# l90lpa/fv3-jedi-linearmodel

Hardware: AMD Instinct MI355X
Metric: column-updates/s per TL+AD dyn step (higher is better)
Workload: dtype f64; 1 GPU; C192L127 hydrostatic TL+AD, six cube faces dealt over 1 GPU(s) (6 per rank), table-driven exchange (221184 columns per GPU), k_split=2 n_split=6 dt=450s nq=4, hord mt/vt/tm/dp/tr=2/2/2/2/2 (sponge: 1/1/1/1 below level 9), kord=17, nord=1; columns_per_gpu=221184

## Files before the change

### fv3_jedi_linearmodel_amd/csrc/remap.h

```cpp
#pragma once
#include "column.h"

namespace fv3 {

struct ColWs {
  double* base; size_t stride; int kw;
  HD double& at(int slot, int k) const { return base[((size_t)slot * kw + k) * stride]; }
};
template <class T> struct WsIO;
template <> struct WsIO<double> {
  static constexpr int W = 1;
  HD static double get(const ColWs& w, int s, int k) { return w.at(s, k); }
  HD static void set(const ColWs& w, int s, int k, double x) { w.at(s, k) = x; }
};
template <> struct WsIO<Dual> {
  static constexpr int W = 2;
  HD static Dual get(const ColWs& w, int s, int k) { return Dual(w.at(2 * s, k), w.at(2 * s + 1, k)); }
  HD static void set(const ColWs& w, int s, int k, const Dual& x) { w.at(2 * s, k) = x.v; w.at(2 * s + 1, k) = x.d; }
};

constexpr double R3 = 1. / 3., R23 = 2. / 3.;

template <class T, class FP1, class FQ1, class FP2, class FOut>
HD void map_col(int km, const FP1& pe1, const FQ1& q1, const FP2& pe2, const FOut& out, const ColWs& ws, int SG, int SE) {
  typedef WsIO<T> W;
  T dpa = pe1(2) - pe1(1), dpb = pe1(3) - pe1(2);
  T grat = dpb / dpa;
  T bet = grat * (grat + 0.5);
  T qf = ((grat + grat) * (grat + 1.) * q1(1) + q1(2)) / bet;
  T gam = (1. + grat * (grat + 1.5)) / bet;
  W::set(ws, SE, 1, qf); W::set(ws, SG, 1, gam);
  T d4 = grat, a_prev = q1(1), dp_prev = dpa;
  for (int k = 2; k <= km; ++k) {
    T dpk = pe1(k + 1) - pe1(k);
    T ak_ = q1(k);
    d4 = dp_prev / dpk;
    bet = 2. + d4 + d4 - gam;
    qf = (3. * (a_prev + d4 * ak_) - qf) / bet;
    gam = d4 / bet;
    W::set(ws, SE, k, qf); W::set(ws, SG, k, gam);
    a_prev = ak_; dp_prev = dpk;
  }
  T a_bot = 1. + d4 * (d4 + 1.5);
  T qe = (2. * d4 * (d4 + 1.) * q1(km) + q1(km - 1) - a_bot * qf) / (d4 * (d4 + 0.5) - a_bot * gam);
  W::set(ws, SE, km + 1, qe);
  for (int k = km; k >= 1; --k) {
    qe = W::get(ws, SE, k) - W::get(ws, SG, k) * qe;
    W::set(ws, SE, k, qe);
  }
  int k0 = 1;
  T qsum = T(0.);
  for (int k = 1; k <= km; ++k) {
    const T p2t = pe2(k), p2b = pe2(k + 1);
    int l; bool found = false;
    for (l = k0; l <= km; ++l)
      if (val(p2t) >= val(pe1(l)) && val(p2t) <= val(pe1(l + 1))) { found = true; break; }
    if (found) {
      const T p1l = pe1(l), p1r = pe1(l + 1), dpl = p1r - p1l;
      const T a1 = q1(l), a2 = W::get(ws, SE, l), a3 = W::get(ws, SE, l + 1), a4 = 3. * (2. * a1 - (a2 + a3));
      const T pl = (p2t - p1l) / dpl;
      if (val(p2b) <= val(p1r)) {
        const T pr = (p2b - p1l) / dpl;
        out(k, a2 + 0.5 * (a4 + a3 - a2) * (pr + pl) - a4 * R3 * (pr * (pr + pl) + pl * pl));
        k0 = l;
        continue;
      }
      qsum = (p1r - p2t) * (a2 + 0.5 * (a4 + a3 - a2) * (1. + pl) - a4 * (R3 * (1. + pl * (1. + pl))));
      int m; bool bottom = false;
      for (m = l + 1; m <= km; ++m) {
        if (val(p2b) > val(pe1(m + 1))) qsum = qsum + (pe1(m + 1) - pe1(m)) * q1(m);
        else { bottom = true; break; }
      }
      if (bottom) {
        const T p1m = pe1(m), dpm = pe1(m + 1) - p1m;
        const T b1 = q1(m), b2 = W::get(ws, SE, m), b3 = W::get(ws, SE, m + 1), b4 = 3. * (2. * b1 - (b2 + b3));
        const T dp = p2b - p1m, esl = dp / dpm;
        qsum = qsum + dp * (b2 + 0.5 * esl * (b3 - b2 + b4 * (1. - R23 * esl)));
        k0 = m;
      }
    }
    out(k, qsum / (p2b - p2t));
  }
}

HD void cs_limiters(bool extm, double a1, double& a2, double& a3, double& a4, int iv) {
  if (iv == 0) {
    if (a1 <= 0.) { a2 = a1; a3 = a1; a4 = 0.; }
    else if (fabs(a3 - a2) < -a4) {
      if (a1 + 0.25 * (a3 - a2) * (a3 - a2) / a4 + a4 * (1. / 12.) < 0.) {
        if (a1 < a3 && a1 < a2) { a3 = a1; a2 = a1; a4 = 0.; }
        else if (a3 > a2) { a4 = 3. * (a2 - a1); a3 = a2 - a4; }
        else { a4 = 3. * (a3 - a1); a2 = a3 - a4; }
      }
    }
    return;
  }
  const bool flat = (iv == 1) ? ((a1 - a2) * (a1 - a3) >= 0.) : extm;
  if (flat) { a2 = a1; a3 = a1; a4 = 0.; return; }
  const double da1 = a3 - a2, da2 = da1 * da1, a6da = a4 * da1;
  if (a6da < -da2) { a4 = 3. * (a2 - a1); a3 = a2 - a4; }
  else if (a6da > da2) { a4 = 3. * (a3 - a1); a2 = a3 - a4; }
}
struct LimProfile { int kord, iv; bool scalar; double qmin; };
template <class FA, class FE>
HD void lim_layer(const LimProfile& P, int k, int km, const FA& a1, const FE& qe, double& a2, double& a3, double& a4) {
  const int ak = P.kord < 0 ? -P.kord : P.kord, iv = P.iv;
  auto qlim = [&](int j) -> double {
    double q = qe(j);
    if (j <= 1 || j >= km + 1) return q;
    const double lo = fmin(a1(j - 1), a1(j)), hi = fmax(a1(j - 1), a1(j));
    if (j == 2 || j == km) return fmax(fmin(q, hi), lo);
    const double g1 = a1(j - 1) - a1(j - 2), g2 = a1(j + 1) - a1(j);
    if (g1 * g2 > 0.) return fmax(fmin(q, hi), lo);
    if (g1 > 0.) return fmax(q, lo);
    q = fmin(q, hi);
    return iv == 0 ? fmax(0., q) : q;
  };
  auto gam = [&](int j) { return a1(j) - a1(j - 1); };
  auto extm = [&](int j) -> bool {
    return gam(j) * gam(j + 1) < 0.;
  };
  const double a = a1(k);
  a2 = qlim(k); a3 = qlim(k + 1);
  if (k == 1 || k == km) {
    const bool ex = (a2 - a) * (a3 - a) > 0.;
    if (k == 1) {
      if (iv == 0) a2 = fmax(0., a2);
      else if (iv == -1) { if (a2 * a <= 0.) a2 = 0.; }
    } else {
      if (iv == 0) a3 = fmax(0., a3);
      else if (iv == -1) { if (a3 * a <= 0.) a3 = 0.; }
    }
    a4 = 3. * (2. * a - (a2 + a3));
    cs_limiters(ex, a, a2, a3, a4, 1);
    return;
  }
  if (k == 2 || k == km - 1) { a4 = 3. * (2. * a - (a2 + a3)); cs_limiters(extm(k), a, a2, a3, a4, 2); return; }
  const bool ex = extm(k), small = P.scalar && a < P.qmin;
  auto huynh = [&]() {
    const double pmp_1 = a - 2. * gam(k + 1), lac_1 = pmp_1 + 1.5 * gam(k + 2);
    a2 = fmin(fmax(a2, fmin(a, fmin(pmp_1, lac_1))), fmax(a, fmax(pmp_1, lac_1)));
    const double pmp_2 = a + 2. * gam(k), lac_2 = pmp_2 - 1.5 * gam(k - 1);
    a3 = fmin(fmax(a3, fmin(a, fmin(pmp_2, lac_2))), fmax(a, fmax(pmp_2, lac_2)));
  };
  if (ak == 9) {
    if (ex && (extm(k - 1) || extm(k + 1) || small)) { a2 = a; a3 = a; a4 = 0.; }
    else {
      a4 = 3. * (2. * a - (a2 + a3));
      if (fabs(a4) > fabs(a2 - a3)) { huynh(); a4 = 3. * (2. * a - (a2 + a3)); }
    }
  } else if (ak == 10) {
    if (ex) {
      if (small || extm(k - 1) || extm(k + 1)) { a2 = a; a3 = a; a4 = 0.; }
      else a4 = 6. * a - 3. * (a2 + a3);
    } else {
      a4 = 6. * a - 3. * (a2 + a3);
      if (fabs(a4) > fabs(a2 - a3)) { huynh(); a4 = 6. * a - 3. * (a2 + a3); }
    }
  } else if (ak == 8) {
    huynh(); a4 = 3. * (2. * a - (a2 + a3));
  } else if (ak == 12) {
    if (ex) { a2 = a; a3 = a; a4 = 0.; }
    else {
      a4 = 6. * a - 3. * (a2 + a3);
      if (fabs(a4) > fabs(a2 - a3)) { huynh(); a4 = 6. * a - 3. * (a2 + a3); }
    }
  } else if (ak == 13) {
    if (ex) {
      if (extm(k - 1) && extm(k + 1)) { a2 = a; a3 = a; a4 = 0.; }
      else { huynh(); a4 = 3. * (2. * a - (a2 + a3)); }
    } else a4 = 3. * (2. * a - (a2 + a3));
  } else if (ak == 14) {
    a4 = 3. * (2. * a - (a2 + a3));
  } else {
    if (ex && (extm(k - 1) || extm(k + 1) || small)) { a2 = a; a3 = a; a4 = 0.; }
    else a4 = 3. * (2. * a - (a2 + a3));
  }
  if (iv == 0) cs_limiters(ex, a, a2, a3, a4, 0);
}
template <class FP1, class FQ1, class FP2, class FE, class FOut>
HD void map_loop_lim(const LimProfile& P, int km, const FP1& pe1, const FQ1& q1, const FP2& pe2, const FE& qe, const FOut& out) {
  int k0 = 1;
  double qsum = 0.;
  for (int k = 1; k <= km; ++k) {
    const double p2t = pe2(k), p2b = pe2(k + 1);
    int l; bool found = false;
    for (l = k0; l <= km; ++l)
      if (p2t >= pe1(l) && p2t <= pe1(l + 1)) { found = true; break; }
    if (found) {
      const double p1l = pe1(l), p1r = pe1(l + 1), dpl = p1r - p1l;
      double a2, a3, a4; lim_layer(P, l, km, q1, qe, a2, a3, a4);
      const double pl = (p2t - p1l) / dpl;
      if (p2b <= p1r) {
        const double pr = (p2b - p1l) / dpl;
        out(k, a2 + 0.5 * (a4 + a3 - a2) * (pr + pl) - a4 * R3 * (pr * (pr + pl) + pl * pl));
        k0 = l;
        continue;
      }
      qsum = (p1r - p2t) * (a2 + 0.5 * (a4 + a3 - a2) * (1. + pl) - a4 * (R3 * (1. + pl * (1. + pl))));
      int m; bool bottom = false;
      for (m = l + 1; m <= km; ++m) {
        if (p2b > pe1(m + 1)) qsum = qsum + (pe1(m + 1) - pe1(m)) * q1(m);
        else { bottom = true; break; }
      }
      if (bottom) {
        const double p1m = pe1(m), dpm = pe1(m + 1) - p1m;
        double b2, b3, b4; lim_layer(P, m, km, q1, qe, b2, b3, b4);
        const double dp = p2b - p1m, esl = dp / dpm;
        qsum = qsum + dp * (b2 + 0.5 * esl * (b3 - b2 + b4 * (1. - R23 * esl)));
        k0 = m;
      }
    }
    out(k, qsum / (p2b - p2t));
  }
}

template <class FP1, class FQ1, class FP2, class FOut>
HD void map_col_lim(const LimProfile& P, int km, const FP1& pe1, const FQ1& q1, const FP2& pe2, const FOut& out, const ColWs& ws, int SG, int SE) {
  {
    double dpa = pe1(2) - pe1(1), dpb = pe1(3) - pe1(2);
    double grat = dpb / dpa, bet = grat * (grat + 0.5);
    double qf = ((grat + grat) * (grat + 1.) * q1(1) + q1(2)) / bet, gam = (1. + grat * (grat + 1.5)) / bet;
    ws.at(SE, 1) = qf; ws.at(SG, 1) = gam;
    double d4 = grat, a_prev = q1(1), dp_prev = dpa;
    for (int k = 2; k <= km; ++k) {
      const double dpk = pe1(k + 1) - pe1(k), ak_ = q1(k);
      d4 = dp_prev / dpk;
      bet = 2. + d4 + d4 - gam;
      qf = (3. * (a_prev + d4 * ak_) - qf) / bet;
      gam = d4 / bet;
      ws.at(SE, k) = qf; ws.at(SG, k) = gam;
      a_prev = ak_; dp_prev = dpk;
    }
    const double a_bot = 1. + d4 * (d4 + 1.5);
    double qe = (2. * d4 * (d4 + 1.) * q1(km) + q1(km - 1) - a_bot * qf) / (d4 * (d4 + 0.5) - a_bot * gam);
// ... 464 lines not shown
  typedef RemapAdSlots R_;
  auto pe1 = [&](int k) { return a.pe.t[fidx(g, a.pe, tile, i, j, k)]; };
  auto pn1 = [&](int k) { return a.peln.t[fidx(g, a.peln, tile, i, j, k)]; };
  auto pk1 = [&](int k) { return a.pk.t[fidx(g, a.pk, tile, i, j, k)]; };
  const double ps = pe1(km + 1);
  auto pe2 = [&](int k) -> double { return k == 1 ? a.ptop : (k == km + 1 ? ps : a.ak[k - 1] + a.bk[k - 1] * ps); };
  auto pn2 = [&](int k) -> double { return (k == 1 || k == km + 1) ? pn1(k) : log(pe2(k)); };
  auto pk2 = [&](int k) -> double { return (k == 1 || k == km + 1) ? pk1(k) : exp(a.akap * pn2(k)); };
  auto ptin = [&](int k) { return a.pt.t[fidx(g, a.pt, tile, i, j, k)]; };
  auto tv = [&](int k) -> double { return ptin(k) * (pk1(k + 1) - pk1(k)) / (a.akap * (pn1(k + 1) - pn1(k))); };
  for (int k = 0; k <= km + 1; ++k)
    for (int s_ : {R_::SPE1, R_::SPN1, R_::SPK1, R_::SPE2, R_::SPN2, R_::SPK2}) ws.at(s_, k) = 0.;
  {
    auto outT = [&](int k, double x) { ws.at(R_::ST2, k) = x; };
    bool done = false;
    if constexpr (LIM) if (kord_limited(a.kord_tm)) { map_col_lim(LimProfile{a.kord_tm, 1, true, 184.}, km, pn1, tv, pn2, outT, ws, 0, 1); done = true; }
    if (!done) map_col<double>(km, pn1, tv, pn2, outT, ws, 0, 1);
    if (a.nq > 0 && a.last_step) {
      auto q1 = [&](int k) { return a.q[0].t[fidx(g, a.q[0], tile, i, j, k)]; };
      auto outQ = [&](int k, double x) { ws.at(R_::SQ2, k) = x; };
      bool doneq = false;
      if constexpr (LIM) if (kord_limited(a.kord_tr)) { map_col_lim(LimProfile{a.kord_tr, 0, true, 0.}, km, pe1, q1, pe2, outQ, ws, 0, 1); doneq = true; }
      if (!doneq) map_col<double>(km, pe1, q1, pe2, outQ, ws, 0, 1);
    }
  }
  for (int k = 1; k <= km; ++k) {
    const size_t n0 = fidx(g, a.pt, tile, i, j, k);
    const double pk_hi = pk2(k), pk_lo = pk2(k + 1), pn_hi = pn2(k), pn_lo = pn2(k + 1);
    const double den = a.akap * (pn_lo - pn_hi), pkz = (pk_lo - pk_hi) / den;
    const double pt_ad = a.pt.p[n0], t2 = ws.at(R_::ST2, k);
    double pkz_ad = a.pkz.p[n0], t2_ad;
    if (a.last_step) {
      const double qv = a.nq > 0 ? ws.at(R_::SQ2, k) : 0., f = 1. + a.zvir * qv;
      t2_ad = pt_ad / f;
      if (a.nq > 0) a.q[0].p[fidx(g, a.q[0], tile, i, j, k)] += -(t2 / f) * a.zvir * pt_ad / f;
    } else {
      t2_ad = pt_ad / pkz;
      pkz_ad += -(t2 / pkz) * pt_ad / pkz;
    }
    ws.at(R_::SV, k) = t2_ad;
    const double za = pkz_ad / den;
    ws.at(R_::SPK2, k + 1) += za; ws.at(R_::SPK2, k) -= za;
    const double zb = -pkz * a.akap * za;
    ws.at(R_::SPN2, k + 1) += zb; ws.at(R_::SPN2, k) -= zb;
    const double dpa = a.delp.p[n0];
    ws.at(R_::SPE2, k + 1) += dpa; ws.at(R_::SPE2, k) -= dpa;
    a.delp.p[n0] = 0.; a.pkz.p[n0] = 0.;
  }
  for (int k = 2; k <= km; ++k) {
    ws.at(R_::SPK2, k) += a.pk.p[fidx(g, a.pk, tile, i, j, k)];
    ws.at(R_::SPN2, k) += a.peln.p[fidx(g, a.peln, tile, i, j, k)];
  }
}
HD void remap_ad_k2(const RemapArgs& a, int field, int i, int j, int tile, size_t col) {
  const Geom& g = a.g; const int km = g.npz;
  const ColWs ws{a.ws + col, a.ws_stride, km + 2};
  const FieldAdSlots S = remap_field_slots(field);
  auto pe1 = [&](int k) { return a.pe.t[fidx(g, a.pe, tile, i, j, k)]; };
  const double ps = pe1(km + 1);
  auto pe2 = [&](int k) -> double { return k == 1 ? a.ptop : (k == km + 1 ? ps : a.ak[k - 1] + a.bk[k - 1] * ps); };
  auto p1out = [&](int k, double x) { ws.at(S.SP1, k) = x; };
  auto p2out = [&](int k, double x) { ws.at(S.SP2, k) = x; };
  if (field == 0) {
    auto pn1 = [&](int k) { return a.peln.t[fidx(g, a.peln, tile, i, j, k)]; };
    auto pk1 = [&](int k) { return a.pk.t[fidx(g, a.pk, tile, i, j, k)]; };
    auto pn2 = [&](int k) -> double { return (k == 1 || k == km + 1) ? pn1(k) : log(pe2(k)); };
    auto tv = [&](int k) -> double { return a.pt.t[fidx(g, a.pt, tile, i, j, k)] * (pk1(k + 1) - pk1(k)) / (a.akap * (pn1(k + 1) - pn1(k))); };
    auto q2ad = [&](int k) { return ws.at(RemapAdSlots::SV, k); };
    map_col_ad_s(km, pn1, tv, pn2, q2ad, ws, S.w, [&](int k, double x) { ws.at(S.SQ1, k) = x; }, p1out, p2out);
  } else {
    const Fld& qf = a.q[field - 1];
    auto q1 = [&](int k) { return qf.t[fidx(g, qf, tile, i, j, k)]; };
    auto q2ad = [&](int k) { return qf.p[fidx(g, qf, tile, i, j, k)]; };
    map_col_ad_s(km, pe1, q1, pe2, q2ad, ws, S.w, [&](int k, double x) { qf.p[fidx(g, qf, tile, i, j, k)] = x; }, p1out, p2out);
  }
}
HD void remap_ad_k3(const RemapArgs& a, int i, int j, int tile, size_t col) {
  const Geom& g = a.g; const int km = g.npz;
  const ColWs ws{a.ws + col, a.ws_stride, km + 2};
  typedef RemapAdSlots R_;
  auto pe1 = [&](int k) { return a.pe.t[fidx(g, a.pe, tile, i, j, k)]; };
  auto pn1 = [&](int k) { return a.peln.t[fidx(g, a.peln, tile, i, j, k)]; };
  auto pk1 = [&](int k) { return a.pk.t[fidx(g, a.pk, tile, i, j, k)]; };
  const double ps = pe1(km + 1);
  auto pe2 = [&](int k) -> double { return k == 1 ? a.ptop : (k == km + 1 ? ps : a.ak[k - 1] + a.bk[k - 1] * ps); };
  auto pn2 = [&](int k) -> double { return (k == 1 || k == km + 1) ? pn1(k) : log(pe2(k)); };
  auto pk2 = [&](int k) -> double { return (k == 1 || k == km + 1) ? pk1(k) : exp(a.akap * pn2(k)); };
  {
    const FieldAdSlots S = remap_field_slots(0);
    for (int k = 1; k <= km + 1; ++k) { ws.at(R_::SPN1, k) += ws.at(S.SP1, k); ws.at(R_::SPN2, k) += ws.at(S.SP2, k); }
    for (int k = 1; k <= km; ++k) {
      const double tv_ad = ws.at(S.SQ1, k), dpk = pk1(k + 1) - pk1(k), den = a.akap * (pn1(k + 1) - pn1(k)), pt0 = a.pt.t[fidx(g, a.pt, tile, i, j, k)];
      a.pt.p[fidx(g, a.pt, tile, i, j, k)] = tv_ad * dpk / den;
      const double za = pt0 * tv_ad / den;
      ws.at(R_::SPK1, k + 1) += za; ws.at(R_::SPK1, k) -= za;
      const double zb = -(pt0 * dpk / den) * a.akap * tv_ad / den;
      ws.at(R_::SPN1, k + 1) += zb; ws.at(R_::SPN1, k) -= zb;
    }
  }
  for (int n = 0; n < a.nq; ++n) {
    const FieldAdSlots S = remap_field_slots(1 + n);
    for (int k = 1; k <= km + 1; ++k) { ws.at(R_::SPE1, k) += ws.at(S.SP1, k); ws.at(R_::SPE2, k) += ws.at(S.SP2, k); }
  }
  for (int k = 2; k <= km; ++k) {
    const double pn_ad = ws.at(R_::SPN2, k) + a.akap * pk2(k) * ws.at(R_::SPK2, k);
    ws.at(R_::SPE2, k) += pn_ad / pe2(k);
  }
  for (int k : {1, km + 1}) {
    ws.at(R_::SPN1, k) += ws.at(R_::SPN2, k) + a.peln.p[fidx(g, a.peln, tile, i, j, k)];
    ws.at(R_::SPK1, k) += ws.at(R_::SPK2, k) + a.pk.p[fidx(g, a.pk, tile, i, j, k)];
  }
  double ps_ad = ws.at(R_::SPE2, km + 1);
  for (int k = 2; k <= km; ++k) ps_ad += a.bk[k - 1] * ws.at(R_::SPE2, k);
  ws.at(R_::SPE1, km + 1) += ps_ad;
  for (int k = 1; k <= km + 1; ++k) {
    a.pk.p[fidx(g, a.pk, tile, i, j, k)] = ws.at(R_::SPK1, k);
    a.peln.p[fidx(g, a.peln, tile, i, j, k)] = ws.at(R_::SPN1, k);
    a.pe.p[fidx(g, a.pe, tile, i, j, k)] += ws.at(R_::SPE1, k);
  }
}

template <int MODE, bool LIM = false>
struct RemapFieldFn {
  RemapArgs a; int nf;
  HD void operator()(int i, int j, int z) const {
    const int tile = z / nf, field = z % nf;
    const size_t col = (size_t)tile * a.g.plane + a.g.idx(i, j);
    if (MODE == MODE_NL) remap_field_col<double, LIM>(a, field, i, j, tile, col);
    else if (MODE == MODE_TL) remap_field_col<Dual, LIM>(a, field, i, j, tile, col);
    else remap_ad_k2(a, field, i, j, tile, col);
  }
};
template <int MODE, bool LIM = false>
struct RemapPressFn {
  RemapArgs a;
  HD void operator()(int i, int j, int z) const {
    const size_t col = (size_t)z * a.g.plane + a.g.idx(i, j);
    if (MODE == MODE_NL) remap_press_col<double>(a, i, j, z);
    else if (MODE == MODE_TL) remap_press_col<Dual>(a, i, j, z);
    else if (MODE == MODE_AD) remap_ad_k1<LIM>(a, i, j, z, col);
    else remap_ad_k3(a, i, j, z, col);
  }
};
template <int MODE, bool LIM = false>
struct RemapWindFn {
  RemapArgs a; int dir;
  HD void operator()(int i, int j, int z) const {
    const size_t col = (size_t)z * a.g.plane + a.g.idx(i, j);
    if (MODE == MODE_NL) remap_wind_col<double, LIM>(a, dir, i, j, z, col);
    else if (MODE == MODE_TL) remap_wind_col<Dual, LIM>(a, dir, i, j, z, col);
    else remap_wind_col_ad(a, dir, i, j, z, col);
  }
};
inline void run_remap_winds(Exec& ex, int mode, const RemapArgs& a, double bytes = 0.) {
  const Geom& g = a.g;
  const Rect U{g.is(), g.ie(), g.js(), g.je() + 1}, V{g.is(), g.ie() + 1, g.js(), g.je()};
  if (kord_limited(a.kord_mt) && mode != MODE_AD) {
    if (mode == MODE_NL) { for_points(ex, U, g.ntile, RemapWindFn<MODE_NL, true>{a, 0}, "remap_wind_lim.nl", bytes); for_points(ex, V, g.ntile, RemapWindFn<MODE_NL, true>{a, 1}, "remap_wind_lim.nl", bytes); }
    else { for_points(ex, U, g.ntile, RemapWindFn<MODE_TL, true>{a, 0}, "remap_wind_lim.tl", bytes); for_points(ex, V, g.ntile, RemapWindFn<MODE_TL, true>{a, 1}, "remap_wind_lim.tl", bytes); }
  }
  else if (mode == MODE_NL) { for_points(ex, U, g.ntile, RemapWindFn<MODE_NL>{a, 0}, "remap_wind.nl", bytes); for_points(ex, V, g.ntile, RemapWindFn<MODE_NL>{a, 1}, "remap_wind.nl", bytes); }
  else if (mode == MODE_TL) { for_points(ex, U, g.ntile, RemapWindFn<MODE_TL>{a, 0}, "remap_wind.tl", bytes); for_points(ex, V, g.ntile, RemapWindFn<MODE_TL>{a, 1}, "remap_wind.tl", bytes); }
  else { for_points(ex, V, g.ntile, RemapWindFn<MODE_AD>{a, 1}, "remap_wind.ad", bytes); for_points(ex, U, g.ntile, RemapWindFn<MODE_AD>{a, 0}, "remap_wind.ad", bytes); }
}
struct RemapGatherFn {
  RemapArgs a;
  HD void operator()(int i, int j, int z) const { remap_pe_gather_ad(a, i, j, z); }
};
struct RemapPeFn {
  RemapArgs a; int mode;
  HD void operator()(int i, int j, int z) const {
    for (int k = 2; k <= a.g.npz; ++k) {
      const size_t n = fidx(a.g, a.pe, z, i, j, k);
      a.pe.t[n] = a.pe2.t[n];
      if (mode == MODE_TL) a.pe.p[n] = a.pe2.p[n];
    }
  }
};

inline int remap_ws_slots(int nq) { return RemapAdSlots::FBASE + RemapAdSlots::FN * (1 + nq); }
inline void run_remap(Exec& ex, int mode, const RemapArgs& a) {
  const Geom& g = a.g;
  const Rect A{g.is(), g.ie(), g.js(), g.je()}, H{g.is() - 1, g.ie() + 1, g.js() - 1, g.je() + 1};
  if (mode != MODE_AD) {
    const double cells = double(g.tx) * g.ty * g.ntile * g.npz, w = mode == MODE_TL ? 2. : 1.;
    const int nf = 1 + a.nq;
    const bool lim = kord_limited(a.kord_tm) || kord_limited(a.kord_tr);
    if (lim && mode == MODE_TL) {
      for_points(ex, A, g.ntile * nf, RemapFieldFn<MODE_TL, true>{a, nf}, "remap_fields_lim.tl", 8. * w * (5. + 2. * a.nq) * cells);
      for_points(ex, A, g.ntile, RemapPressFn<MODE_TL>{a}, "remap_press.tl", 8. * w * (5. + 7.) * cells);
    } else if (lim) {
      for_points(ex, A, g.ntile * nf, RemapFieldFn<MODE_NL, true>{a, nf}, "remap_fields_lim.nl", 8. * w * (5. + 2. * a.nq) * cells);
      for_points(ex, A, g.ntile, RemapPressFn<MODE_NL>{a}, "remap_press.nl", 8. * w * (5. + 7.) * cells);
    } else if (mode == MODE_TL) {
      for_points(ex, A, g.ntile * nf, RemapFieldFn<MODE_TL>{a, nf}, "remap_fields.tl", 8. * w * (5. + 2. * a.nq) * cells);
      for_points(ex, A, g.ntile, RemapPressFn<MODE_TL>{a}, "remap_press.tl", 8. * w * (5. + 7.) * cells);
    } else {
      for_points(ex, A, g.ntile * nf, RemapFieldFn<MODE_NL>{a, nf}, "remap_fields.nl", 8. * w * (5. + 2. * a.nq) * cells);
      for_points(ex, A, g.ntile, RemapPressFn<MODE_NL>{a}, "remap_press.nl", 8. * w * (5. + 7.) * cells);
    }
    run_remap_winds(ex, mode, a, 8. * w * 4. * cells);
    for_points(ex, A, g.ntile, RemapPeFn{a, mode}, "remap_pe");
  } else {
    const double cells = double(g.tx) * g.ty * g.ntile * g.npz;
    run_remap_winds(ex, MODE_AD, a, 8. * 7. * cells);
    for_points(ex, H, g.ntile, RemapGatherFn{a}, "remap_gather.ad", 8. * 4. * cells);
    const int nf = 1 + a.nq;
    if (kord_limited(a.kord_tm) || kord_limited(a.kord_tr)) for_points(ex, A, g.ntile, RemapPressFn<MODE_AD, true>{a}, "remap_scalars1_lim.ad", 8. * 12. * cells);
    else for_points(ex, A, g.ntile, RemapPressFn<MODE_AD>{a}, "remap_scalars1.ad", 8. * 12. * cells);
    for_points(ex, A, g.ntile * nf, RemapFieldFn<MODE_AD>{a, nf}, "remap_fields.ad", 8. * (4. + 3. * a.nq) * cells);
    for_points(ex, A, g.ntile, RemapPressFn<3>{a}, "remap_scalars3.ad", 8. * 8. * cells);
  }
}

}
```

Measured before the change: 184,400 column-updates/s.

## Split vertical remap into edge-solve and LDS-staged parallel per-level mapping kernels

Splits the per-column PPM remap for the NL/TL paths into two kernels: one computes edge values (batching up to four tracers per thread and sharing the tridiagonal coefficients), and one stages pressure, field and edge arrays for a strip of columns in LDS. In the second kernel, threads map each target level independently via binary search, so the serial per-column search loop goes away. Columns whose source or target pressures are not monotonic fall back to the serial mapping loop. This adds extra launches, workspace traffic and barrier synchronisation, in exchange for more parallelism and coalesced loads in the mapping step.

```diff
diff --git a/fv3_jedi_linearmodel_amd/csrc/remap.h b/fv3_jedi_linearmodel_amd/csrc/remap.h
--- a/fv3_jedi_linearmodel_amd/csrc/remap.h
+++ b/fv3_jedi_linearmodel_amd/csrc/remap.h
@@ -21,8 +21,8 @@
 
 constexpr double R3 = 1. / 3., R23 = 2. / 3.;
 
-template <class T, class FP1, class FQ1, class FP2, class FOut>
-HD void map_col(int km, const FP1& pe1, const FQ1& q1, const FP2& pe2, const FOut& out, const ColWs& ws, int SG, int SE) {
+template <class T, class FP1, class FQ1>
+HD void map_edges(int km, const FP1& pe1, const FQ1& q1, const ColWs& ws, int SG, int SE) {
   typedef WsIO<T> W;
   T dpa = pe1(2) - pe1(1), dpb = pe1(3) - pe1(2);
   T grat = dpb / dpa;
@@ -48,6 +48,81 @@
     qe = W::get(ws, SE, k) - W::get(ws, SG, k) * qe;
     W::set(ws, SE, k, qe);
   }
+}
+template <class T, int N, class FP1, class FQ1>
+HD void map_edges_n(int km, int nact, const FP1& pe1, const FQ1& q1, const ColWs& ws, int SG, int SE0) {
+  typedef WsIO<T> W;
+  T dpa = pe1(2) - pe1(1), dpb = pe1(3) - pe1(2);
+  T grat = dpb / dpa;
+  T bet = grat * (grat + 0.5);
+  T gam = (1. + grat * (grat + 1.5)) / bet;
+  T qf[N], a_prev[N];
+#pragma unroll
+  for (int n = 0; n < N; ++n) if (n < nact) {
+    a_prev[n] = q1(n, 1);
+    qf[n] = ((grat + grat) * (grat + 1.) * a_prev[n] + q1(n, 2)) / bet;
+    W::set(ws, SE0 + n, 1, qf[n]);
+  }
+  W::set(ws, SG, 1, gam);
+  T d4 = grat, dp_prev = dpa;
+  for (int k = 2; k <= km; ++k) {
+    T dpk = pe1(k + 1) - pe1(k);
+    d4 = dp_prev / dpk;
+    bet = 2. + d4 + d4 - gam;
+#pragma unroll
+    for (int n = 0; n < N; ++n) if (n < nact) {
+      T ak_ = q1(n, k);
+      qf[n] = (3. * (a_prev[n] + d4 * ak_) - qf[n]) / bet;
+      W::set(ws, SE0 + n, k, qf[n]);
+      a_prev[n] = ak_;
+    }
+    gam = d4 / bet;
+    W::set(ws, SG, k, gam);
+    dp_prev = dpk;
+  }
+  T a_bot = 1. + d4 * (d4 + 1.5);
+  T qe[N];
+#pragma unroll
+  for (int n = 0; n < N; ++n) if (n < nact) {
+    qe[n] = (2. * d4 * (d4 + 1.) * q1(n, km) + q1(n, km - 1) - a_bot * qf[n]) / (d4 * (d4 + 0.5) - a_bot * gam);
+    W::set(ws, SE0 + n, km + 1, qe[n]);
+  }
+  for (int k = km; k >= 1; --k) {
+    const T g = W::get(ws, SG, k);
+#pragma unroll
+    for (int n = 0; n < N; ++n) if (n < nact) {
+      qe[n] = W::get(ws, SE0 + n, k) - g * qe[n];
+      W::set(ws, SE0 + n, k, qe[n]);
+    }
+  }
+}
+template <class T, class FP1, class FQ1, class FSE>
+HD T map_target(int km, int l, const T& p2t, const T& p2b, const FP1& pe1, const FQ1& q1, const FSE& se, T& qsum, int& k0) {
+  const T p1l = pe1(l), p1r = pe1(l + 1), dpl = p1r - p1l;
+  const T a1 = q1(l), a2 = se(l), a3 = se(l + 1), a4 = 3. * (2. * a1 - (a2 + a3));
+  const T pl = (p2t - p1l) / dpl;
+  if (val(p2b) <= val(p1r)) {
+    const T pr = (p2b - p1l) / dpl;
+    k0 = l;
+    return a2 + 0.5 * (a4 + a3 - a2) * (pr + pl) - a4 * R3 * (pr * (pr + pl) + pl * pl);
+  }
+  qsum = (p1r - p2t) * (a2 + 0.5 * (a4 + a3 - a2) * (1. + pl) - a4 * (R3 * (1. + pl * (1. + pl))));
+  int m; bool bottom = false;
+  for (m = l + 1; m <= km; ++m) {
+    if (val(p2b) > val(pe1(m + 1))) qsum = qsum + (pe1(m + 1) - pe1(m)) * q1(m);
+    else { bottom = true; break; }
+  }
+  if (bottom) {
+    const T p1m = pe1(m), dpm = pe1(m + 1) - p1m;
+    const T b1 = q1(m), b2 = se(m), b3 = se(m + 1), b4 = 3. * (2. * b1 - (b2 + b3));
+    const T dp = p2b - p1m, esl = dp / dpm;
+    qsum = qsum + dp * (b2 + 0.5 * esl * (b3 - b2 + b4 * (1. - R23 * esl)));
+    k0 = m;
+  }
+  return qsum / (p2b - p2t);
+}
+template <class T, class FP1, class FQ1, class FP2, class FSE, class FOut>
+HD void map_loop(int km, const FP1& pe1, const FQ1& q1, const FP2& pe2, const FSE& se, const FOut& out) {
   int k0 = 1;
   T qsum = T(0.);
   for (int k = 1; k <= km; ++k) {
@@ -55,32 +130,14 @@
     int l; bool found = false;
     for (l = k0; l <= km; ++l)
       if (val(p2t) >= val(pe1(l)) && val(p2t) <= val(pe1(l + 1))) { found = true; break; }
-    if (found) {
-      const T p1l = pe1(l), p1r = pe1(l + 1), dpl = p1r - p1l;
-      const T a1 = q1(l), a2 = W::get(ws, SE, l), a3 = W::get(ws, SE, l + 1), a4 = 3. * (2. * a1 - (a2 + a3));
-      const T pl = (p2t - p1l) / dpl;
-      if (val(p2b) <= val(p1r)) {
-        const T pr = (p2b - p1l) / dpl;
-        out(k, a2 + 0.5 * (a4 + a3 - a2) * (pr + pl) - a4 * R3 * (pr * (pr + pl) + pl * pl));
-        k0 = l;
-        continue;
-      }
-      qsum = (p1r - p2t) * (a2 + 0.5 * (a4 + a3 - a2) * (1. + pl) - a4 * (R3 * (1. + pl * (1. + pl))));
-      int m; bool bottom = false;
-      for (m = l + 1; m <= km; ++m) {
-        if (val(p2b) > val(pe1(m + 1))) qsum = qsum + (pe1(m + 1) - pe1(m)) * q1(m);
-        else { bottom = true; break; }
-      }
-      if (bottom) {
-        const T p1m = pe1(m), dpm = pe1(m + 1) - p1m;
-        const T b1 = q1(m), b2 = W::get(ws, SE, m), b3 = W::get(ws, SE, m + 1), b4 = 3. * (2. * b1 - (b2 + b3));
-        const T dp = p2b - p1m, esl = dp / dpm;
-        qsum = qsum + dp * (b2 + 0.5 * esl * (b3 - b2 + b4 * (1. - R23 * esl)));
-        k0 = m;
-      }
-    }
-    out(k, qsum / (p2b - p2t));
-  }
+    if (found) out(k, map_target<T>(km, l, p2t, p2b, pe1, q1, se, qsum, k0));
+    else out(k, qsum / (p2b - p2t));
+  }
+}
+template <class T, class FP1, class FQ1, class FP2, class FOut>
+HD void map_col(int km, const FP1& pe1, const FQ1& q1, const FP2& pe2, const FOut& out, const ColWs& ws, int SG, int SE) {
+  map_edges<T>(km, pe1, q1, ws, SG, SE);
+  map_loop<T>(km, pe1, q1, pe2, [&](int k) { return WsIO<T>::get(ws, SE, k); }, out);
 }
 
 HD void cs_limiters(bool extm, double a1, double& a2, double& a3, double& a4, int iv) {
@@ -851,8 +908,13 @@
     else remap_wind_col_ad(a, dir, i, j, z, col);
   }
 };
+}
+#include "remap_split.h"
+namespace fv3 {
+
 inline void run_remap_winds(Exec& ex, int mode, const RemapArgs& a, double bytes = 0.) {
   const Geom& g = a.g;
+  if (mode != MODE_AD && !kord_limited(a.kord_mt) && run_remap_winds_split(ex, mode, a, bytes)) return;
   const Rect U{g.is(), g.ie(), g.js(), g.je() + 1}, V{g.is(), g.ie() + 1, g.js(), g.je()};
   if (kord_limited(a.kord_mt) && mode != MODE_AD) {
     if (mode == MODE_NL) { for_points(ex, U, g.ntile, RemapWindFn<MODE_NL, true>{a, 0}, "remap_wind_lim.nl", bytes); for_points(ex, V, g.ntile, RemapWindFn<MODE_NL, true>{a, 1}, "remap_wind_lim.nl", bytes); }
@@ -885,7 +947,10 @@
     const double cells = double(g.tx) * g.ty * g.ntile * g.npz, w = mode == MODE_TL ? 2. : 1.;
     const int nf = 1 + a.nq;
     const bool lim = kord_limited(a.kord_tm) || kord_limited(a.kord_tr);
-    if (lim && mode == MODE_TL) {
+    if (!lim && run_remap_fields_split(ex, mode, a, cells)) {
+      if (mode == MODE_TL) for_points(ex, A, g.ntile, RemapPressFn<MODE_TL>{a}, "remap_press.tl", 8. * w * (5. + 7.) * cells);
+      else for_points(ex, A, g.ntile, RemapPressFn<MODE_NL>{a}, "remap_press.nl", 8. * w * (5. + 7.) * cells);
+    } else if (lim && mode == MODE_TL) {
       for_points(ex, A, g.ntile * nf, RemapFieldFn<MODE_TL, true>{a, nf}, "remap_fields_lim.tl", 8. * w * (5. + 2. * a.nq) * cells);
       for_points(ex, A, g.ntile, RemapPressFn<MODE_TL>{a}, "remap_press.tl", 8. * w * (5. + 7.) * cells);
     } else if (lim) {
diff --git a/fv3_jedi_linearmodel_amd/csrc/remap_split.h b/fv3_jedi_linearmodel_amd/csrc/remap_split.h
--- /dev/null
+++ b/fv3_jedi_linearmodel_amd/csrc/remap_split.h
@@ -0,0 +1,259 @@
+#pragma once
+
+namespace fv3 {
+
+constexpr int RS_NT = 4;
+constexpr int RS_NTH = 512;
+constexpr int RS_CMAX = 64;
+inline bool remap_split_enabled() { const char* e = std::getenv("FV3LM_REMAP_SPLIT"); return !(e && e[0] == '0'); }
+inline size_t remap_split_lds(int npz, int C, bool tl) { return (size_t)3 * (npz + 2) * C * (tl ? 16 : 8); }
+inline int remap_split_cols(int npz, bool tl) {
+  int C = RS_CMAX;
+  while (C >= 8 && remap_split_lds(npz, C, tl) > 160 * 1024) C /= 2;
+  while (C >= 16 && remap_split_lds(npz, C, tl) > 53 * 1024) C /= 2;
+  return C >= 8 ? C : 0;
+}
+
+template <class T_>
+struct RsTv {
+  typedef T_ T; typedef FIO<T> IO;
+  const RemapArgs& a; int i, j, tile;
+  HD RsTv(const RemapArgs& a_, int, int i_, int j_, int tile_) : a(a_), i(i_), j(j_), tile(tile_) {}
+  HD static int nfld(const RemapArgs&) { return 1; }
+  HD static int slot_e(const RemapArgs&, int, int) { return 1; }
+  HD T pn1(int k) const { return IO::ld(a.peln, fidx(a.g, a.peln, tile, i, j, k)); }
+  HD T pk1(int k) const { return IO::ld(a.pk, fidx(a.g, a.pk, tile, i, j, k)); }
+  HD T pe1(int k) const { return pn1(k); }
+  HD T q1(int, int k) const { return IO::ld(a.pt, fidx(a.g, a.pt, tile, i, j, k)) * (pk1(k + 1) - pk1(k)) / (a.akap * (pn1(k + 1) - pn1(k))); }
+  HD T surf() const { return IO::ld(a.pe, fidx(a.g, a.pe, tile, i, j, a.g.npz + 1)); }
+  HD T pe2p(int k, const T& ps) const { const int km = a.g.npz; return k == 1 ? T(a.ptop) : (k == km + 1 ? ps : a.ak[k - 1] + a.bk[k - 1] * ps); }
+  HD T pe2(int k, const T& ps) const { return (k == 1 || k == a.g.npz + 1) ? pn1(k) : dlog(pe2p(k, ps)); }
+  HD void st(int, int k, const T& x) const { IO::st(a.pt, fidx(a.g, a.pt, tile, i, j, k), x); }
+};
+template <class T_>
+struct RsTr {
+  typedef T_ T; typedef FIO<T> IO;
+  const RemapArgs& a; int i, j, tile;
+  HD RsTr(const RemapArgs& a_, int, int i_, int j_, int tile_) : a(a_), i(i_), j(j_), tile(tile_) {}
+  HD static int nfld(const RemapArgs& a_) { return a_.nq; }
+  HD static int slot_e(const RemapArgs&, int, int n) { return 2 + n; }
+  HD T pe1(int k) const { return IO::ld(a.pe, fidx(a.g, a.pe, tile, i, j, k)); }
+  HD Fld qn(int n) const {
+    Fld f = a.q[0];
+#pragma unroll
+    for (int m = 1; m < 8; ++m) if (m == n) f = a.q[m];
+    return f;
+  }
+  HD T q1(int n, int k) const { const Fld f = qn(n); return IO::ld(f, fidx(a.g, f, tile, i, j, k)); }
+  HD T surf() const { return pe1(a.g.npz + 1); }
+  HD T pe2(int k, const T& ps) const { const int km = a.g.npz; return k == 1 ? T(a.ptop) : (k == km + 1 ? ps : a.ak[k - 1] + a.bk[k - 1] * ps); }
+  HD void st(int n, int k, const T& x) const { const Fld f = qn(n); IO::st(f, fidx(a.g, f, tile, i, j, k), x); }
+};
+template <class T_>
+struct RsWind {
+  typedef T_ T; typedef FIO<T> IO;
+  const RemapArgs& a; int dir, i, j, tile, im, jm;
+  HD RsWind(const RemapArgs& a_, int dir_, int i_, int j_, int tile_) : a(a_), dir(dir_), i(i_), j(j_), tile(tile_), im(dir_ == 0 ? i_ : i_ - 1), jm(dir_ == 0 ? j_ - 1 : j_) {}
+  HD static int nfld(const RemapArgs&) { return 1; }
+  HD static int slot_e(const RemapArgs&, int dir_, int) { return 2 * dir_ + 1; }
+  HD const Fld& wf() const { return dir == 0 ? a.u : a.v; }
+  HD T pe1(int k) const {
+    if (k == 1) return IO::ld(a.pe, fidx(a.g, a.pe, tile, i, j, 1));
+    return 0.5 * (IO::ld(a.pe, fidx(a.g, a.pe, tile, im, jm, k)) + IO::ld(a.pe, fidx(a.g, a.pe, tile, i, j, k)));
+  }
+  HD T q1(int, int k) const { return IO::ld(wf(), fidx(a.g, wf(), tile, i, j, k)); }
+  HD T surf() const { const int km = a.g.npz; return IO::ld(a.pe, fidx(a.g, a.pe, tile, im, jm, km + 1)) + IO::ld(a.pe, fidx(a.g, a.pe, tile, i, j, km + 1)); }
+  HD T pe2(int k, const T& pss) const { return (dir == 1 && k == 1) ? T(a.ak[0]) : a.ak[k - 1] + (0.5 * a.bk[k - 1]) * pss; }
+  HD void st(int, int k, const T& x) const { IO::st(wf(), fidx(a.g, wf(), tile, i, j, k), x); }
+};
+HD Rect remap_wind_rect(const Geom& g, int dir) { return dir == 0 ? Rect{g.is(), g.ie(), g.js(), g.je() + 1} : Rect{g.is(), g.ie() + 1, g.js(), g.je()}; }
+
+template <class T>
+struct RemapEdgesFieldFn {
+  RemapArgs a; int ng;
+  HD void operator()(int i, int j, int z) const {
+    const int tile = z / ng, grp = z % ng, km = a.g.npz;
+    const ColWs ws{a.ws + (size_t)tile * a.g.plane + a.g.idx(i, j), a.ws_stride, km + 2};
+    if (grp == 0) {
+      const RsTv<T> p(a, 0, i, j, tile);
+      map_edges<T>(km, [&](int k) { return p.pe1(k); }, [&](int k) { return p.q1(0, k); }, ws, 0, 1);
+    } else {
+      const RsTr<T> p(a, 0, i, j, tile);
+      const int n0 = RS_NT * (grp - 1), nact = a.nq - n0 < RS_NT ? a.nq - n0 : RS_NT;
+      map_edges_n<T, RS_NT>(km, nact, [&](int k) { return p.pe1(k); }, [&](int n, int k) { return p.q1(n0 + n, k); }, ws, 2 + a.nq + (grp - 1), 2 + n0);
+    }
+  }
+};
+template <class T>
+struct RemapEdgesWindFn {
+  RemapArgs a;
+  HD void operator()(int i, int j, int z) const {
+    const int tile = z / 2, dir = z % 2, km = a.g.npz;
+    if (!remap_wind_rect(a.g, dir).has(i, j)) return;
+    const ColWs ws{a.ws + (size_t)tile * a.g.plane + a.g.idx(i, j), a.ws_stride, km + 2};
+    const RsWind<T> p(a, dir, i, j, tile);
+    map_edges<T>(km, [&](int k) { return p.pe1(k); }, [&](int k) { return p.q1(0, k); }, ws, 2 * dir, 2 * dir + 1);
+  }
+};
+
+#ifdef FV3LM_HOST_EMUL
+DEV void rs_sync() {}
+#else
+DEV void rs_sync() { __syncthreads(); }
+#endif
+template <int U, class T, class FL, class FS>
+DEV void rs_stage(int n, int tid, int nth, const FL& ld, const FS& st) {
+  for (int e0 = tid; e0 < n; e0 += U * nth) {
+    T v[U];
+#pragma unroll
+    for (int u = 0; u < U; ++u) { const int e = e0 + u * nth; if (e < n) v[u] = ld(e); }
+#pragma unroll
+    for (int u = 0; u < U; ++u) { const int e = e0 + u * nth; if (e < n) st(e, v[u]); }
+  }
+}
+template <class PL>
+DEV void remap_map_block(const RemapArgs& a, int sel, const Rect& R, int tile, int j, int i0, int C, unsigned char* mem, int tid, int nth) {
+  typedef typename PL::T T; typedef WsIO<T> W;
+  const int km = a.g.npz, nc = R.i1 - i0 + 1 < C ? R.i1 - i0 + 1 : C, nf = PL::nfld(a);
+  int lc = 0; while ((1 << lc) < C) ++lc;
+  constexpr int U = sizeof(T) == 8 ? 8 : 4;
+  T* const P = reinterpret_cast<T*>(mem);
+  T* const Q = P + (size_t)(km + 1) * C;
+  T* const E = Q + (size_t)km * C;
+  int* const bad = reinterpret_cast<int*>(E + (size_t)(km + 1) * C);
+  for (int e = tid; e < C; e += nth) bad[e] = 0;
+  rs_stage<U, T>((km + 1) * C, tid, nth, [&](int e) { const int c = e & (C - 1); return c < nc ? PL(a, sel, i0 + c, j, tile).pe1(1 + (e >> lc)) : T(0.); },
+                 [&](int e, const T& x) { P[e] = x; });
+  rs_sync();
+  for (int e = tid; e < km * C; e += nth) {
+    const int c = e & (C - 1), k = 1 + (e >> lc);
+    if (c >= nc) continue;
+    const PL p(a, sel, i0 + c, j, tile);
+    const T s = p.surf(), p2t = p.pe2(k, s), p2b = p.pe2(k + 1, s);
+    bool ok = val(P[k * C + c]) > val(P[(k - 1) * C + c]) && val(p2b) >= val(p2t);
+    if (k == 1) ok = ok && val(p2t) >= val(P[c]);
+    if (k == km) ok = ok && val(p2t) <= val(P[km * C + c]);
+    if (!ok) bad[c] = 1;
+  }
+  for (int n = 0; n < nf; ++n) {
+    if (n > 0) rs_sync();
+    const int SE = PL::slot_e(a, sel, n);
+    rs_stage<U, T>((km + 1) * C, tid, nth, [&](int e) {
+                     const int c = e & (C - 1);
+                     if (c >= nc) return T(0.);
+                     return W::get(ColWs{a.ws + (size_t)tile * a.g.plane + a.g.idx(i0 + c, j), a.ws_stride, km + 2}, SE, 1 + (e >> lc)); },
+                   [&](int e, const T& x) { E[e] = x; });
+    rs_stage<U, T>(km * C, tid, nth, [&](int e) { const int c = e & (C - 1); return c < nc ? PL(a, sel, i0 + c, j, tile).q1(n, 1 + (e >> lc)) : T(0.); },
+                   [&](int e, const T& x) { Q[e] = x; });
+    rs_sync();
+    for (int e = tid; e < km * C; e += nth) {
+      const int c = e & (C - 1), k = 1 + (e >> lc);
+      if (c >= nc) continue;
+      const PL p(a, sel, i0 + c, j, tile);
+      auto pe1 = [&](int kk) { return P[(kk - 1) * C + c]; };
+      auto q1 = [&](int kk) { return Q[(kk - 1) * C + c]; };
+      auto se = [&](int kk) { return E[(kk - 1) * C + c]; };
+      if (bad[c]) {
+        if (k == 1) {
+          const T s = p.surf();
+          map_loop<T>(km, pe1, q1, [&](int kk) { return p.pe2(kk, s); }, se, [&](int kk, const T& x) { p.st(n, kk, x); });
+        }
+        continue;
+      }
+      const T s = p.surf(), p2t = p.pe2(k, s), p2b = p.pe2(k + 1, s);
+      int lo = 1, hi = km;
+      while (lo < hi) {
+        const int mid = (lo + hi) >> 1;
+        if (val(p2t) <= val(P[mid * C + c])) hi = mid; else lo = mid + 1;
+      }
+      T qsum = T(0.); int k0;
+      p.st(n, k, map_target<T>(km, lo, p2t, p2b, pe1, q1, se, qsum, k0));
+    }
+  }
+}
+template <class T, int KIND>
+DEV void remap_map_dispatch(const RemapArgs& a, int bx, int by, int z, int C, unsigned char* mem, int tid, int nth) {
+  const Geom& g = a.g;
+  if (KIND != 1) {
+    const int tile = z;
+    const Rect R{g.is(), g.ie(), g.js(), g.je()};
+    const int i0 = R.i0 + bx * C, j = R.j0 + by;
+    if (i0 > R.i1 || j > R.j1) return;
+    if (KIND == 0) remap_map_block<RsTv<T>>(a, 0, R, tile, j, i0, C, mem, tid, nth);
+    else remap_map_block<RsTr<T>>(a, 0, R, tile, j, i0, C, mem, tid, nth);
+  } else {
+    const int tile = z / 2, dir = z % 2;
+    const Rect R = remap_wind_rect(g, dir);
+    const int i0 = R.i0 + bx * C, j = R.j0 + by;
+    if (i0 > R.i1 || j > R.j1) return;
+    remap_map_block<RsWind<T>>(a, dir, R, tile, j, i0, C, mem, tid, nth);
+  }
+}
+#ifndef FV3LM_HOST_EMUL
+template <class T, int KIND>
+__global__ void __launch_bounds__(RS_NTH) k_remap_map(RemapArgs a, int C) {
+  extern __shared__ __attribute__((aligned(16))) unsigned char rs_lds[];
+  int bx = blockIdx.x, by = blockIdx.y; xcd_block(gridDim.x, gridDim.y, bx, by);
+  remap_map_dispatch<T, KIND>(a, bx, by, blockIdx.z, C, rs_lds, threadIdx.x, RS_NTH);
+}
+#endif
+template <int KIND>
+inline void launch_remap_map(Exec& ex, int mode, const RemapArgs& a, int C, const char* name, double bytes) {
+  const Geom& g = a.g;
+  const bool tl = mode == MODE_TL;
+  const int nx = g.tx + (KIND == 1), ny = g.ty + (KIND == 1), nbx = (nx + C - 1) / C, nz = g.ntile * (KIND == 1 ? 2 : 1);
+  const size_t lds = remap_split_lds(g.npz, C, tl);
+  ex.mark_begin(name, "", bytes);
+#ifdef FV3LM_HOST_EMUL
+  std::vector<double> mem((lds + 7) / 8);
+  for (int z = 0; z < nz; ++z)
+    for (int by = 0; by < ny; ++by)
+      for (int bx = 0; bx < nbx; ++bx) {
+        if (tl) remap_map_dispatch<Dual, KIND>(a, bx, by, z, C, reinterpret_cast<unsigned char*>(mem.data()), 0, 1);
+        else remap_map_dispatch<double, KIND>(a, bx, by, z, C, reinterpret_cast<unsigned char*>(mem.data()), 0, 1);
+      }
+#else
+  static bool attr = false;
+  if (!attr) {
+    const int cap = 160 * 1024;
+    if (hipFuncSetAttribute((const void*)k_remap_map<double, 0>, hipFuncAttributeMaxDynamicSharedMemorySize, cap) != hipSuccess ||
+        hipFuncSetAttribute((const void*)k_remap_map<double, 1>, hipFuncAttributeMaxDynamicSharedMemorySize, cap) != hipSuccess ||
+        hipFuncSetAttribute((const void*)k_remap_map<Dual, 0>, hipFuncAttributeMaxDynamicSharedMemorySize, cap) != hipSuccess ||
+        hipFuncSetAttribute((const void*)k_remap_map<Dual, 1>, hipFuncAttributeMaxDynamicSharedMemorySize, cap) != hipSuccess ||
+        hipFuncSetAttribute((const void*)k_remap_map<double, 2>, hipFuncAttributeMaxDynamicSharedMemorySize, cap) != hipSuccess ||
+        hipFuncSetAttribute((const void*)k_remap_map<Dual, 2>, hipFuncAttributeMaxDynamicSharedMemorySize, cap) != hipSuccess) set_sticky("hipFuncSetAttribute(k_remap_map) failed");
+    attr = true;
+  }
+  const dim3 grid(nbx, ny, nz);
+  if (tl) hipLaunchKernelGGL((k_remap_map<Dual, KIND>), grid, dim3(RS_NTH), lds, ex.stream, a, C);
+  else hipLaunchKernelGGL((k_remap_map<double, KIND>), grid, dim3(RS_NTH), lds, ex.stream, a, C);
+#endif
+  ex.mark_end();
+  ex.launches++;
+}
+
+inline bool run_remap_winds_split(Exec& ex, int mode, const RemapArgs& a, double bytes) {
+  const int C = remap_split_enabled() ? remap_split_cols(a.g.npz, mode == MODE_TL) : 0;
+  if (!C) return false;
+  const Geom& g = a.g;
+  const Rect UV{g.is(), g.ie() + 1, g.js(), g.je() + 1};
+  if (mode == MODE_TL) for_points(ex, UV, g.ntile * 2, RemapEdgesWindFn<Dual>{a}, "remap_edges.tl", 2. * bytes * 0.75);
+  else for_points(ex, UV, g.ntile * 2, RemapEdgesWindFn<double>{a}, "remap_edges.nl", 2. * bytes * 0.75);
+  launch_remap_map<1>(ex, mode, a, C, mode == MODE_TL ? "remap_map.tl" : "remap_map.nl", 2. * bytes * 0.25);
+  return true;
+}
+inline bool run_remap_fields_split(Exec& ex, int mode, const RemapArgs& a, double cells) {
+  const int C = remap_split_enabled() ? remap_split_cols(a.g.npz, mode == MODE_TL) : 0;
+  if (!C) return false;
+  const Geom& g = a.g;
+  const Rect A{g.is(), g.ie(), g.js(), g.je()};
+  const int ng = 1 + (a.nq + RS_NT - 1) / RS_NT;
+  const double w = mode == MODE_TL ? 2. : 1.;
+  if (mode == MODE_TL) for_points(ex, A, g.ntile * ng, RemapEdgesFieldFn<Dual>{a, ng}, "remap_edges.tl", 8. * w * (4. + a.nq) * cells);
+  else for_points(ex, A, g.ntile * ng, RemapEdgesFieldFn<double>{a, ng}, "remap_edges.nl", 8. * w * (4. + a.nq) * cells);
+  launch_remap_map<0>(ex, mode, a, C, mode == MODE_TL ? "remap_map.tl" : "remap_map.nl", 8. * w * cells);
+  if (a.nq > 0) launch_remap_map<2>(ex, mode, a, C, mode == MODE_TL ? "remap_map.tl" : "remap_map.nl", 8. * w * a.nq * cells);
+  return true;
+}
+
+}
```

Result: no change. 186,200 column-updates/s, median of 6 (+0.9%).
